# danielmtzbarba/carlabev-env

Measured on NVIDIA B200. Metric: env-steps/sec (obs+reward+done) at N envs, 1/2/4/8 B200; % HBM roofline, higher is better.
Workload: dtype f64

## Files before the change

### carlabev_env_b200/csrc/api.cu

```cuda
#include <cuda.h>
#include <math.h>
#include <stdarg.h>
#include <stdio.h>
#include <stdlib.h>
#include <string.h>

#include <algorithm>
#include <chrono>
#include <cmath>
#include <new>
#include <random>
#include <vector>

#include "engine.h"

static thread_local char g_err[512] = "";

void cbev_set_error(const char* fmt, ...) {
  va_list ap;
  va_start(ap, fmt);
  vsnprintf(g_err, sizeof(g_err), fmt, ap);
  va_end(ap);
}

// ... 344 lines not shown
  else e->frame_bytes = (int64_t)cfg->fov_size * cfg->fov_size * 3;

  const size_t N = (size_t)e->N, A = (size_t)(cfg->max_actors > 0 ? cfg->max_actors : 1);
  int rc = 0;
  rc |= dev_alloc(&e->st.scene, N);
  rc |= dev_alloc(&e->st.episode, N);
  rc |= dev_alloc(&e->st.done, N);
  rc |= dev_alloc(&e->st.ego, N * 24);
  rc |= dev_alloc(&e->st.egoi, N * 8);
  rc |= dev_alloc(&e->st.tgt_vis, N * CBEV_TGT_WORDS);
  rc |= dev_alloc(&e->st.stats, N * 12);
  rc |= dev_alloc(&e->st.ax, N * A);
  rc |= dev_alloc(&e->st.ay, N * A);
  rc |= dev_alloc(&e->st.ayaw, N * A);
  rc |= dev_alloc(&e->st.av, N * A);
  rc |= dev_alloc(&e->st.atarget_mps, N * A);
  rc |= dev_alloc(&e->st.aelapsed, N * A);
  rc |= dev_alloc(&e->st.astate_elapsed, N * A);
  rc |= dev_alloc(&e->st.atidx, N * A);
  rc |= dev_alloc(&e->st.arxlen, N * A);
  rc |= dev_alloc(&e->st.aflags, N * A);
  rc |= dev_alloc(&e->desc, N * CBEV_DESC_WORDS);
  rc |= dev_alloc(&e->order, N);
  rc |= dev_alloc(&e->order_cnt, (size_t)2);
  rc |= dev_alloc(&e->move_order, N);
  rc |= dev_alloc(&e->move_cnt, (size_t)2);
  rc |= dev_alloc(&e->fov, N * (size_t)cfg->fov_size * cfg->fov_size);
  rc |= dev_alloc(&e->gstats, (size_t)CBEV_STATS_FIELDS);
  rc |= build_resize_tables(e);
  rc |= dev_alloc((uint8_t**)&e->h_reward_dev, N * 10);
  e->h_term_dev = (uint8_t*)e->h_reward_dev + N * 8;
  e->h_trunc_dev = e->h_term_dev + N;
  rc |= dev_alloc((uint8_t**)&e->h_actions_dev, N * 16);
  if (rc) { cbev_destroy(e); return rc; }
  cudaMemset(e->st.scene, 0xff, N * sizeof(int32_t));
  {
    uint64_t z = (uint64_t)std::chrono::steady_clock::now().time_since_epoch().count() ^ (uint64_t)(uintptr_t)e;
    try {
      std::random_device rd;
      z ^= ((uint64_t)rd() << 32) | (uint64_t)rd();
    } catch (...) {
    }
    z += 0x9E3779B97F4A7C15ull;
    z = (z ^ (z >> 30)) * 0xBF58476D1CE4E5B9ull;
    z = (z ^ (z >> 27)) * 0x94D049BB133111EBull;
    e->token = z ^ (z >> 31);
  }
  *out = e;
  return CBEV_OK;
}

int cbev_destroy(cbev_handle e) {
  if (!e) return CBEV_OK;
  use_device(e);
  free_pool(e->pool);
  free_state(e->st);
  free_state(e->branch);
  dev_free(e->br_stage_desc); dev_free(e->br_stage_rects); dev_free(e->br_desc); dev_free(e->br_rects);
  dev_free(e->br_window);
  dev_free(e->fov_mask); dev_free(e->rs_tab); dev_free(e->trace);
  dev_free(e->order); dev_free(e->order_cnt); dev_free(e->move_order); dev_free(e->move_cnt);
  dev_free(e->map); dev_free(e->desc); dev_free(e->rects); dev_free(e->fov); dev_free(e->gstats);
  dev_free(e->h_reward_dev);
  { uint8_t* p = (uint8_t*)e->h_actions_dev; dev_free(p); }
  if (e->side_stream) cudaStreamDestroy(e->side_stream);
  if (e->ev_sim) cudaEventDestroy(e->ev_sim);
  if (e->ev_copy) cudaEventDestroy(e->ev_copy);
  if (e->ev_judge) cudaEventDestroy(e->ev_judge);
  if (e->prof_ev) {
    for (int i = 0; i < CBEV_PROF_EVENTS * CBEV_PROF_MAX; ++i) cudaEventDestroy(e->prof_ev[i]);
    delete[] e->prof_ev;
  }
  delete e;
  return CBEV_OK;
}

int cbev_upload_map(cbev_handle e, const uint8_t* cls_host, int32_t w, int32_t h_px) {
  if (!e || !cls_host) { cbev_set_error("null argument"); return CBEV_ERR_ARG; }
  { int rc0 = use_device(e); if (rc0) return rc0; }
  if (w < 16 || h_px < 16 || (w % 16) != 0) { cbev_set_error("map width must be a multiple of 16 (TMA row pitch), got %dx%d", w, h_px); return CBEV_ERR_ARG; }
  for (size_t i = 0; i < (size_t)w * h_px; ++i)
    if (cls_host[i] > 2) { cbev_set_error("map classes must be 0 (non-drivable), 1 (drivable) or 2 (sidewalk)"); return CBEV_ERR_ARG; }
  dev_free(e->map);
  int rc = dev_upload(&e->map, cls_host, (size_t)w * h_px);
// ... 798 lines not shown
    std::vector<int32_t> ti(N * A);
    std::vector<uint8_t> fl(N * A);
    for (size_t i = 0; i < N * A; ++i) {
      const double* o = actors_host + i * 8;
      x[i] = o[0]; y[i] = o[1]; yaw[i] = o[2]; v[i] = o[3];
      ti[i] = (int32_t)o[4];
      tm[i] = o[6];
      fl[i] = (uint8_t)(((int)o[7] & ~15) | ((int)o[5] & 15));
    }
    CU_TRY(cudaMemcpy(e->st.ax, x.data(), N * A * 8, cudaMemcpyHostToDevice));
    CU_TRY(cudaMemcpy(e->st.ay, y.data(), N * A * 8, cudaMemcpyHostToDevice));
    CU_TRY(cudaMemcpy(e->st.ayaw, yaw.data(), N * A * 8, cudaMemcpyHostToDevice));
    CU_TRY(cudaMemcpy(e->st.av, v.data(), N * A * 8, cudaMemcpyHostToDevice));
    CU_TRY(cudaMemcpy(e->st.atarget_mps, tm.data(), N * A * 8, cudaMemcpyHostToDevice));
    CU_TRY(cudaMemcpy(e->st.atidx, ti.data(), N * A * 4, cudaMemcpyHostToDevice));
    CU_TRY(cudaMemcpy(e->st.aflags, fl.data(), N * A, cudaMemcpyHostToDevice));
  }
  return CBEV_OK;
}

int cbev_set_debug_flags(cbev_handle e, int32_t flags) {
  if (!e) { cbev_set_error("null handle"); return CBEV_ERR_ARG; }
  if (flags & ~CBEV_DBG_KNOWN) {
    cbev_set_error("unknown debug flags 0x%x (accepted bits: 1, 2, 4, 32, 128, 256, 512)",
                   (unsigned)(flags & ~CBEV_DBG_KNOWN));
    return CBEV_ERR_ARG;
  }
  e->debug_flags = flags;
  if ((flags & CBEV_DBG_TRACE) && !e->trace) return dev_alloc(&e->trace, (size_t)e->N * 8);
  return CBEV_OK;
}

int cbev_debug_read_trace(cbev_handle e, uint64_t* host_out) {
  if (!e || !host_out) { cbev_set_error("null argument"); return CBEV_ERR_ARG; }
  { int rc0 = use_device(e); if (rc0) return rc0; }
  if (!e->trace) { cbev_set_error("tracing is off (set debug flag 4 first)"); return CBEV_ERR_STATE; }
  CU_TRY(cudaDeviceSynchronize());
  CU_TRY(cudaMemcpy(host_out, e->trace, (size_t)e->N * 8 * sizeof(uint64_t), cudaMemcpyDeviceToHost));
  return CBEV_OK;
}

int cbev_keep_fov(cbev_handle e, int32_t on) {
  if (!e) { cbev_set_error("null handle"); return CBEV_ERR_ARG; }
  e->keep_fov = on != 0;
  return CBEV_OK;
}

int cbev_copy_fov(cbev_handle e, uint8_t* fov_dev, void* stream) {
  if (!e || !fov_dev) { cbev_set_error("null argument"); return CBEV_ERR_ARG; }
  { int rc0 = use_device(e); if (rc0) return rc0; }
  if (!e->keep_fov) { cbev_set_error("palette frames are not kept: call cbev_keep_fov(h, 1) before stepping"); return CBEV_ERR_STATE; }
  size_t bytes = (size_t)e->N * e->cfg.fov_size * e->cfg.fov_size;
  CU_TRY(cudaMemcpyAsync(fov_dev, e->fov, bytes, cudaMemcpyDeviceToDevice, (cudaStream_t)stream));
  return CBEV_OK;
}

int cbev_read_stats(cbev_handle e, double* stats_dev, int32_t reset_after, void* stream) {
  if (!e || !stats_dev) { cbev_set_error("null argument"); return CBEV_ERR_ARG; }
  { int rc0 = use_device(e); if (rc0) return rc0; }
// ... 64 lines not shown
```

### carlabev_env_b200/csrc/engine.h

```cpp
#pragma once
#include <cuda_runtime.h>
#include <stdint.h>

#include "../../include/cbev.h"

#define CBEV_TGT_WORDS 2
#define CBEV_MAX_TARGETS (64 * CBEV_TGT_WORDS)
#define CBEV_RECT_WORDS 2
#define CBEV_DESC_WORDS 20
#define CBEV_TILE_H 184
#define CBEV_TILE_W 208
#define CBEV_WARPS_PER_BLOCK 4
#define CBEV_PROF_MAX 2048
#define CBEV_PROF_EVENTS 5

enum {
  RD_OX = 0,
  RD_OY,
  RD_MODE,
  RD_TURNS,
  RD_NX, RD_NY, RD_ISIN, RD_ICOS, RD_AX, RD_AY, RD_XD, RD_YD, RD_CY,
  RD_NRECTS,
  RD_FLAGS,
  RD_FX, RD_FY,
// ... 70 lines not shown
  float hero_scale;
  int32_t action_mode, n_discrete, reward_mode, autoreset;
  uint64_t seed;
  const uint8_t* map;
  float discrete_table[16 * 3];
  cbev_config cfg;
};

#define CBEV_RS_FAST96 0
#define CBEV_RS_TABLE 1
#define CBEV_RS_HALF 2
#define CBEV_RS_COPY 3
#define CBEV_RS_LINEAR 4
#define CBEV_ANY_BOX_W 128

enum {
  CBEV_DBG_GENERIC_ROTATE = 1,
  CBEV_DBG_JUDGE_SERIAL = 2,
  CBEV_DBG_TRACE = 4,
  CBEV_DBG_IDENTITY_RENDER_ORDER = 32,
  CBEV_DBG_IDENTITY_MOVE_ORDER = 128,
  CBEV_DBG_RENDER_ANY = 256,
  CBEV_DBG_NO_BLOCK83 = 512,
  CBEV_DBG_KNOWN = CBEV_DBG_GENERIC_ROTATE | CBEV_DBG_JUDGE_SERIAL | CBEV_DBG_TRACE | CBEV_DBG_IDENTITY_RENDER_ORDER |
                   CBEV_DBG_IDENTITY_MOVE_ORDER | CBEV_DBG_RENDER_ANY | CBEV_DBG_NO_BLOCK83
};

struct cbev_engine {
  cbev_config cfg;
  int device = 0;
  int32_t N = 0, crop = 0, pad = 0, anchor_x = 0, anchor_y = 0;
  int32_t map_w = 0, map_h = 0;
  uint8_t* map = nullptr;
  alignas(64) unsigned char tmap[128];
  alignas(64) unsigned char tmap_any[128];
  int32_t win_max = 0;
  int32_t any_nbx = 0, any_nby = 0, any_box_h = 0;
  bool has_map = false, has_pool = false, was_reset = false, keep_fov = false;
  PoolDev pool;
  EnvState st;
  int32_t max_rects = 0;
  int32_t debug_flags = 0;
  int32_t* desc = nullptr;
  uint32_t* rects = nullptr;
  int32_t* order = nullptr;
  int32_t* order_cnt = nullptr;
  int32_t* move_order = nullptr;
  int32_t* move_cnt = nullptr;
  uint8_t* fov = nullptr;
  unsigned long long* trace = nullptr;
  int32_t rs_mode = 0, rs_words = 0;
  int32_t* rs_tab = nullptr;
  uint8_t* fov_mask = nullptr;
  void* ring = nullptr;
  int64_t ring_bytes = 0, frame_bytes = 0;
  int32_t channels = 0;
  int32_t head = -1;
  double* gstats = nullptr;
  void* h_actions_dev = nullptr;
  double* h_reward_dev = nullptr;
  uint8_t *h_term_dev = nullptr, *h_trunc_dev = nullptr;
  cudaStream_t side_stream = nullptr;
  cudaEvent_t ev_sim = nullptr, ev_copy = nullptr, ev_judge = nullptr;
  bool host_copy_pending = false;
  int64_t launches = 0;
  int64_t steps = 0;
  bool profiling = false;
  cudaEvent_t* prof_ev = nullptr;
  int32_t prof_n = 0;
// ... 46 lines not shown
```

### carlabev_env_b200/csrc/render.cu

```cuda
#include <cuda.h>
#include <stdlib.h>

#include <type_traits>

#include "engine.h"

namespace {

constexpr int RT = 256;

__constant__ uint32_t c_pal_rg[CBEV_PAL_COUNT];
__constant__ uint32_t c_pal_b[CBEV_PAL_COUNT];
__constant__ uint32_t c_pal_key[CBEV_PAL_COUNT];
__constant__ uint8_t c_chan_mask[6][CBEV_PAL_COUNT + 1];

__device__ __forceinline__ uint32_t smem_u32(const void* p) { return (uint32_t)__cvta_generic_to_shared(p); }

__device__ __forceinline__ void mbar_init(uint64_t* bar, int count) {
  asm volatile("mbarrier.init.shared::cta.b64 [%0], %1;" ::"r"(smem_u32(bar)), "r"(count));
}
__device__ __forceinline__ void mbar_expect_tx(uint64_t* bar, uint32_t bytes) {
  asm volatile("mbarrier.arrive.expect_tx.shared::cta.b64 _, [%0], %1;" ::"r"(smem_u32(bar)), "r"(bytes) : "memory");
}
__device__ __forceinline__ void mbar_wait(uint64_t* bar, uint32_t parity) {
// ... 22 lines not shown
__device__ __forceinline__ uint32_t bit_to_f32(uint32_t m, int pos) {
  int32_t s;
  asm("bfe.s32 %0, %1, %2, 1;" : "=r"(s) : "r"(m), "r"(pos));
  return (uint32_t)s & 0x3f800000u;
}
__device__ __forceinline__ void st_b4(void* p, uint32_t a, uint32_t b, uint32_t c, uint32_t d) {
  asm volatile("st.global.cs.v4.b32 [%0], {%1, %2, %3, %4};" ::"l"(p), "r"(a), "r"(b), "r"(c), "r"(d) : "memory");
}
__device__ __forceinline__ void st_u4(void* p, uint4 v) {
  asm volatile("st.global.cs.v4.u32 [%0], {%1, %2, %3, %4};" ::"l"(p), "r"(v.x), "r"(v.y), "r"(v.z), "r"(v.w)
               : "memory");
}

struct RenderParams {
  int32_t N, fov, crop, anchor_x, anchor_y;
  int32_t frame_stack, ring_slots, head, mirror;
  int64_t frame_bytes;
  int32_t generic_rotate;
  int32_t blk83;
  int32_t list_cap;
  const int32_t* desc;
  const uint32_t* rects;
  const int32_t* order;
  int32_t* order_cnt;
  int32_t max_rects;
  uint8_t* fov_out;
  const uint8_t* fov_mask;
  void* ring;
  int32_t obs_h, obs_w, rs_mode, rs_words;
  const int32_t* rs_tab;
  unsigned long long* trace;
  int32_t hero_w;
  int32_t nbx, nby, box_h, region_bytes;
};

__device__ __forceinline__ void trace_mark(const RenderParams& P, int env, int slot) {
  if (P.trace != nullptr && threadIdx.x == 0) {
    unsigned long long t;
    asm volatile("mov.u64 %0, %%globaltimer;" : "=l"(t));
    P.trace[(size_t)env * 8 + slot] = t;
    if (slot == 0) {
      unsigned sm;
      asm volatile("mov.u32 %0, %%smid;" : "=r"(sm));
      P.trace[(size_t)env * 8 + 6] = sm;
    }
  }
}
// ... 65 lines not shown

template <int OBS_MODE, int CHANNELS, bool U8 = false>
__global__ void __launch_bounds__(RT, 4)
k_render(RenderParams P, const __grid_constant__ CUtensorMap tmap, int mask_mode) {
  extern __shared__ __align__(128) uint8_t smem[];
  constexpr int S = 128;
  constexpr int pitch = CBEV_TILE_W;
  constexpr int tile_bytes = CBEV_TILE_W * CBEV_TILE_H;
  uint8_t* s_tile = smem;
  uint8_t* const s_region = smem;
  uint8_t* s_fov = smem + tile_bytes;
  uint32_t* s_rg = (uint32_t*)(s_fov + S * S);
  uint32_t* s_b = s_rg + 16;
  uint32_t* s_key = s_b + 16;
  int32_t* s_desc = (int32_t*)(s_key + 16);
  uint64_t* s_bar = (uint64_t*)(s_desc + CBEV_DESC_WORDS);
  uint8_t* s_cm = (uint8_t*)(s_bar + 2);
  int* s_count = (int*)(s_cm + 16);
  uint32_t* s_rects = (uint32_t*)(s_count + 4);

  const int env = P.order != nullptr ? P.order[blockIdx.x] : blockIdx.x;
  const int tid = threadIdx.x;
  const int lane = tid & 31, warp = tid >> 5;
  if (blockIdx.x == 0 && tid < 2 && P.order_cnt != nullptr) P.order_cnt[tid] = 0;
  const int32_t* d = P.desc + (size_t)env * CBEV_DESC_WORDS;
  const int flags = d[RD_FLAGS];
  if (flags & 2) return;
  trace_mark(P, env, 0);

  if (tid == 0) {
    mbar_init(s_bar, 1);
    asm volatile("fence.mbarrier_init.release.cluster;" ::: "memory");
    mbar_expect_tx(s_bar, (uint32_t)tile_bytes);
    tma_load_2d(s_tile, &tmap, d[RD_OX] & ~15, d[RD_OY], s_bar);
    *s_count = 0;
  }
  if (tid < CBEV_DESC_WORDS) s_desc[tid] = d[tid];
  if (tid < CBEV_PAL_COUNT) {
    s_rg[tid] = c_pal_rg[tid];
    s_b[tid] = c_pal_b[tid];
    s_key[tid] = c_pal_key[tid];
  }
  if (tid <= CBEV_PAL_COUNT) s_cm[tid] = c_chan_mask[mask_mode][tid];
  const int nrects = d[RD_NRECTS];
  {
    const uint32_t* rl = P.rects + (size_t)env * P.max_rects * CBEV_RECT_WORDS;
    for (int r = tid; r < P.max_rects * CBEV_RECT_WORDS; r += RT) s_rects[r] = rl[r];
// ... 271 lines not shown
  const int S = P.fov, NT = blockDim.x;
  const int FP = S + 16;
  constexpr int BW = CBEV_ANY_BOX_W;
  const int tile_h = P.box_h * P.nby;
  const int tile_bytes = BW * P.nbx * tile_h;
  uint8_t* const s_tile = smem;
  uint8_t* const s_fov = smem + P.region_bytes;
  uint32_t* s_rg = (uint32_t*)(s_fov + S * FP);
  uint32_t* s_b = s_rg + 16;
  uint32_t* s_key = s_b + 16;
  int32_t* s_desc = (int32_t*)(s_key + 16);
  uint64_t* s_bar = (uint64_t*)(s_desc + CBEV_DESC_WORDS);
  uint8_t* s_cm = (uint8_t*)(s_bar + 2);
  uint8_t* s_cmu = s_cm + 16;
  float4* s_palf = (float4*)(s_cmu + 16);
  uint32_t* s_rects = (uint32_t*)(s_palf + 16);
  int32_t* s_tab = (int32_t*)(s_rects + ((P.max_rects * CBEV_RECT_WORDS + 3) & ~3));
  uint8_t* s_bflag = (uint8_t*)(s_tab + P.rs_words);
  uint8_t* s_out_sep = s_bflag + ((((S >> 3) * (S >> 3)) + 15) & ~15);

  const int env = P.order != nullptr ? P.order[blockIdx.x] : blockIdx.x;
  const int tid = threadIdx.x;
  const int lane = tid & 31, warp = tid >> 5, nwarps = NT >> 5;
  if (blockIdx.x == 0 && tid < 2 && P.order_cnt != nullptr) P.order_cnt[tid] = 0;
  const int32_t* d = P.desc + (size_t)env * CBEV_DESC_WORDS;
  const int flags = d[RD_FLAGS];
  if (flags & 2) return;
  trace_mark(P, env, 0);

  if (tid == 0) {
    mbar_init(s_bar, 1);
    asm volatile("fence.mbarrier_init.release.cluster;" ::: "memory");
    mbar_expect_tx(s_bar, (uint32_t)tile_bytes);
    const int x0 = d[RD_OX] & ~15, y0 = d[RD_OY];
    for (int bx = 0; bx < P.nbx; ++bx)
      for (int by = 0; by < P.nby; ++by)
        tma_load_2d(s_tile + (size_t)(bx * tile_h + by * P.box_h) * BW, &tmap, x0 + bx * BW, y0 + by * P.box_h, s_bar);
  }
  if (tid < CBEV_DESC_WORDS) s_desc[tid] = d[tid];
  if (tid < CBEV_PAL_COUNT) {
    s_rg[tid] = c_pal_rg[tid];
    s_b[tid] = c_pal_b[tid];
    s_key[tid] = c_pal_key[tid];
  }
  if (tid <= CBEV_PAL_COUNT) s_cm[tid] = c_chan_mask[mask_mode][tid];
  const int nrects = d[RD_NRECTS];
  {
// ... 641 lines not shown
                   e->max_rects);
    return 1;
  }
  int rc = 1;
  if (e->cfg.obs_mode == CBEV_OBS_RGB) rc = launch<CBEV_OBS_RGB, 1>(e, P, smem, smem_any, any, s);
  else if (e->cfg.obs_mode == CBEV_OBS_GRAY) rc = launch<CBEV_OBS_GRAY, 1>(e, P, smem, smem_any, any, s);
  else if (e->cfg.obs_mode == CBEV_OBS_SEMANTIC_U8) rc = launch_semantic<true>(e, P, smem, smem_any, any, s);
  else rc = launch_semantic<false>(e, P, smem, smem_any, any, s);
  if (rc == 0) e->launches += 1;
  return rc;
}

}

int cbev_launch_render(cbev_engine* e, int32_t head, int32_t mirror, cudaStream_t s) {
  RenderParams P;
  P.N = e->N;
  P.ring_slots = e->cfg.ring_slots;
  P.head = head;
  P.mirror = mirror;
  P.desc = e->desc;
  P.rects = e->rects;
  P.order = (e->debug_flags & CBEV_DBG_IDENTITY_RENDER_ORDER) ? nullptr : e->order;
  P.order_cnt = e->order_cnt;
  P.fov_out = e->keep_fov ? e->fov : nullptr;
  P.ring = e->ring;
  P.trace = (e->debug_flags & CBEV_DBG_TRACE) ? e->trace : nullptr;
  return render_launch(e, P, s);
}

int cbev_launch_render_branches(cbev_engine* e, int32_t n, void* windows, cudaStream_t s) {
  RenderParams P;
  P.N = n;
  P.ring_slots = 1;
  P.head = 0;
  P.mirror = 0;
  P.desc = e->br_desc;
  P.rects = e->br_rects;
  P.order = nullptr;
  P.order_cnt = nullptr;
  P.fov_out = nullptr;
  P.ring = windows;
  P.trace = nullptr;
  return render_launch(e, P, s);
}

int cbev_launch_fuse(cbev_engine* e, int32_t mode, const void* ring, int32_t n, int32_t L, int32_t head, void* out,
                     cudaStream_t s) {
  static const int veh_of[6] = {-1, -1, 1, 2, 3, 3};
  const int veh = veh_of[e->cfg.mask_mode];
  if (veh < 0) return 1;
  const int C = e->channels;
  const int Cout = mode == CBEV_FUSE_VEHICLE_TEMPORAL ? C - 1 + 3 : C;
  const bool u8 = e->cfg.obs_mode == CBEV_OBS_SEMANTIC_U8;
  const int HWV = e->cfg.obs_h * e->cfg.obs_w / (u8 ? 16 : 4);
  long long total = (long long)n * Cout * HWV;
  int blocks = (int)((total + 255) / 256);
  if (blocks > 148 * 32) blocks = 148 * 32;
  if (!u8)
    k_fuse<<<blocks, 256, 0, s>>>((const float4*)ring, (float*)out, n, L, C, head, veh, mode, HWV);
  else if (mode == CBEV_FUSE_VEHICLE_TEMPORAL)
    k_fuse<<<blocks, 256, 0, s>>>((const uint4*)ring, (uint8_t*)out, n, L, C, head, veh, mode, HWV);
  else
// ... 5 lines not shown
```

### carlabev_env_b200/csrc/sim.cu

```cuda
#include <limits.h>
#include <math.h>

#include "engine.h"

#ifndef CBEV_SIM_BLOCKS_PER_SM
#define CBEV_SIM_BLOCKS_PER_SM 7
#endif

namespace {

constexpr double DT = 0.1;
constexpr double WB = 2.9;
constexpr double KST = 2.0;
constexpr double KPS = 1.0;
constexpr double MPP = 0.3125;
constexpr double MAX_STEER = 0x1.0c152382d7365p-1;
constexpr double PI = 0x1.921fb54442d18p+1;
constexpr double TWO_PI = 0x1.921fb54442d18p+2;
constexpr double HALF_PI = 0x1.921fb54442d18p+0;
constexpr double DEG2RAD = 0x1.1df46a2529d39p-6;
constexpr double RAD2DEG = 0x1.ca5dc1a63c1f8p+5;
constexpr unsigned FULL = 0xffffffffu;

enum { E_X = 0, E_Y, E_YAW, E_V, E_X1, E_Y1, E_YAW1, E_V1, E_ACC, E_T, E_D2G, E_D2G1, E_SPREV, E_LAST_DYAW,
// ... 495 lines not shown
__device__ __forceinline__ void live_actor_chunk(const SimParams& P, const PoolDev& pool, const EnvState& S, size_t row, int ga,
                                              size_t o, bool has, double t_sim, int lane, int gb, unsigned GM, Body& b,
                                              int& kind) {
  actor_chunk_step<G>(P, pool, S, row, ga, o, has, t_sim, lane, gb, GM, b, kind);
}

template <int G>
__device__ __forceinline__ void hand_over_to_live(const SimParams& P, const PoolDev& pool, const EnvState& st, int env, int scene,
                                               int A, int lane, unsigned GM) {
  for (int a = lane; a < A; a += G) {
    const size_t o = (size_t)env * P.max_actors + a, r = (size_t)scene * P.max_actors + a;
    st.ax[o] = pool.roll.ax[r]; st.ay[o] = pool.roll.ay[r]; st.ayaw[o] = pool.roll.ayaw[r]; st.av[o] = pool.roll.av[r];
    st.atarget_mps[o] = pool.roll.atarget_mps[r]; st.aelapsed[o] = pool.roll.aelapsed[r];
    st.astate_elapsed[o] = pool.roll.astate_elapsed[r]; st.atidx[o] = pool.roll.atidx[r];
    st.arxlen[o] = pool.roll.arxlen[r]; st.aflags[o] = pool.roll.aflags[r];
  }
  for (int k = lane; k < P.max_retreat * 3 * CBEV_SG_MAX; k += G)
    st.retreat[(size_t)env * P.max_retreat * 3 * CBEV_SG_MAX + k] = pool.roll.retreat[(size_t)scene * P.max_retreat * 3 * CBEV_SG_MAX + k];
  for (int k = lane; k < P.max_retreat; k += G)
    st.retreat_n[(size_t)env * P.max_retreat + k] = pool.roll.retreat_n[(size_t)scene * P.max_retreat + k];
  __syncwarp(GM);
}

template <int G>
__device__ __forceinline__ void auto_reset_env(const SimParams& P, const PoolDev& pool, const EnvState& st, const cbev_step_out& out,
                                            int32_t* d, int32_t* order, int32_t* order_cnt, int env, int lane, unsigned GM) {
  int ep = st.episode[env];
  uint64_t h = splitmix64(P.seed + (uint64_t)env * 0x9E3779B97F4A7C15ull + (uint64_t)ep * 0xD1B54A32D192ED03ull);
  int scene = (int)(h % (uint64_t)pool.n_scenes);
  __syncwarp(GM);
  reset_env(P, pool, st, env, scene, lane, G);
  if (lane == 0) {
    order[atomicAdd(order_cnt, 1)] = env;
    const double* s0 = pool.ego_state0 + (size_t)scene * 4;
    View v;
    compute_view(P, s0[0], s0[1], 0.0, v);
    write_desc_header(P, d, v, 0, 1, crop_corner_class(P, v));
    out.reward[env] = 0.0;
    out.terminated[env] = 0;
    out.truncated[env] = 0;
    if (out.cause) out.cause[env] = CBEV_CAUSE_NONE;
    if (out.hero) {
      double* hb = out.hero + (size_t)env * CBEV_HERO_FIELDS;
      for (int k = 0; k < CBEV_HERO_FIELDS; ++k) hb[k] = 0.0;
      hb[CBEV_H_X] = s0[0]; hb[CBEV_H_Y] = s0[1]; hb[CBEV_H_YAW] = s0[2]; hb[CBEV_H_V] = s0[3];
      hb[CBEV_H_SCENE] = (double)scene;
    }
  }
}

template <int G>
struct Group {
  int warp, lane, gb, grp;
  unsigned GM;
  int env;
  __device__ __forceinline__ Group(const SimParams& P, const int32_t* __restrict__ perm = nullptr) {
    constexpr int EPW = 32 / G;
    warp = threadIdx.x >> 5;
    const int wl = threadIdx.x & 31;
    lane = wl & (G - 1);
    gb = wl & ~(G - 1);
    grp = wl / G;
    GM = G == 32 ? 0xffffffffu : (((1u << G) - 1u) << gb);
    env = (blockIdx.x * CBEV_WARPS_PER_BLOCK + warp) * EPW + grp;
    if (perm != nullptr && env < P.N) env = perm[env];
  }
};

enum { MV_LIVE = 0, MV_BRANCH = 1, MV_BRANCH_DRAW = 2 };
template <int G, int MODE>
__device__ __forceinline__ void move_body(const SimParams& P, const PoolDev& pool, const EnvState& st,
                                          const void* __restrict__ actions, const cbev_step_out& out,
                                          int32_t* __restrict__ desc, uint32_t* __restrict__ rects,
                                          int32_t* __restrict__ order, int32_t* __restrict__ order_cnt, int env,
                                          int lane, int gb, unsigned GM) {
  constexpr bool BRANCH = MODE != MV_LIVE, DRAW = MODE != MV_BRANCH;
  int32_t* d = desc + (size_t)env * CBEV_DESC_WORDS;
  uint32_t* rl = rects + (size_t)env * P.max_rects * CBEV_RECT_WORDS;

  const uint8_t was_done = BRANCH ? 0 : st.done[env];
  const int scene = st.scene[env];
  double* eg = st.ego + (size_t)env * E_SLOTS;
  const int32_t* ei = st.egoi + (size_t)env * I_SLOTS;
  Body e;
  e.x = eg[E_X]; e.y = eg[E_Y]; e.yaw = eg[E_YAW]; e.v = eg[E_V];
  double acc = eg[E_ACC];
  const double etarget = eg[E_TARGET];
  const double t_sim = eg[E_T] + DT;
  const int step_idx = ei[I_STEP];
  const unsigned long long tv0 = st.tgt_vis[(size_t)env * CBEV_TGT_WORDS], tv1 = st.tgt_vis[(size_t)env * CBEV_TGT_WORDS + 1];
  float gas, steer, brake;
  if (P.action_mode == CBEV_ACTION_DISCRETE) {
    long long id = ((const long long*)actions)[env];
    const int nd = P.n_discrete;
    id = id < 0 ? 0 : (id >= nd ? nd - 1 : id);
    gas = P.discrete_table[id * 3 + 0];
    steer = P.discrete_table[id * 3 + 1];
    brake = P.discrete_table[id * 3 + 2];
  } else {
    const float* a = (const float*)actions + (size_t)env * 3;
    gas = fminf(fmaxf(a[0], 0.0f), 1.0f);
    steer = fminf(fmaxf(a[1], -1.0f), 1.0f);
    brake = fminf(fmaxf(a[2], 0.0f), 1.0f);
  }

  if constexpr (!BRANCH) {
    if (P.autoreset == CBEV_AUTORESET_NEXT_STEP && was_done) {
      auto_reset_env<G>(P, pool, st, out, d, order, order_cnt, env, lane, GM);
      return;
    }
  }

  const int r0 = pool.ego_off[scene], nt = pool.ego_off[scene + 1] - r0;
  const int A0 = pool.actor_off[scene], A = pool.actor_off[scene + 1] - A0;
  const int tl0 = pool.tl_off[scene], ntl = pool.tl_off[scene + 1] - tl0;
  const bool use_table = step_idx < pool.traj_steps;
  const long long toff = pool.traj_steps > 0 ? pool.traj_off[scene] : 0;
  const double* __restrict__ ecx = pool.ego_cx + r0;
  const double* __restrict__ ecy = pool.ego_cy + r0;

  double acc_val = gas > 0.0f ? (double)__fmul_rn(gas, P.hero_scale) : 0.0;
  double delta;
  if (fabs(e.v) < 0.1) {
    delta = 0.0;
  } else {
    double steer_deg = clipd(18.0 / (1.0 + 0.35 * fabs(e.v)), 8.0, 18.0);
    delta = ((double)steer * steer_deg) * DEG2RAD;
  }
  double speed_factor = clipd(fabs(e.v) / 5.0, 0.3, 1.0);
  double brake_val = (brake > 0.0f ? (double)__fmul_rn(__fmul_rn(brake, 0.6f), P.hero_scale) : 0.0) * speed_factor;
  double target_acc = acc_val - brake_val - 0.05 * e.v;
  acc = (1.0 - 0.2) * acc + 0.2 * target_acc;
  const double applied_delta = delta;
  body_update(e, acc, delta, etarget);
  e.v *= 0.9999;
  if (fabs(e.v) < 0.05) e.v = 0.0;
  e.v *= 0.985;
  if (lane == 0) {
    eg[E_X] = e.x; eg[E_Y] = e.y; eg[E_YAW] = e.yaw; eg[E_V] = e.v;
    eg[E_X1] = e.x1; eg[E_Y1] = e.y1; eg[E_YAW1] = e.yaw1; eg[E_V1] = e.v1;
    eg[E_ACC] = acc;
    eg[E_GAS] = (double)gas; eg[E_STEER] = (double)steer; eg[E_BRAKE] = (double)brake; eg[E_DELTA] = applied_delta;
  }

  const int pad = P.pad;
  View view;
  int bg = 0;
  if constexpr (DRAW) {
    compute_view(P, e.x, e.y, e.yaw, view);
    bg = crop_corner_class(P, view);
  }

  int nrects = 0;
  if (!use_table && pool.traj_steps > 0 && step_idx == pool.traj_steps) hand_over_to_live<G>(P, pool, st, env, scene, A, lane, GM);
  double4 qn = make_double4(0.0, 0.0, 0.0, 0.0);
  int kn = 0;
  if (use_table && lane < A) {
    qn = pool.traj[toff + (size_t)step_idx * A + lane];
    kn = pool.act_kind[A0 + lane];
  }
  for (int base = 0; base < A; base += G) {
    const int a = base + lane;
    const bool has = a < A;
    const int ga = A0 + (has ? a : 0);
    const size_t o = (size_t)env * P.max_actors + (has ? a : 0);
    Body b;
    int kind = 0;
    if (use_table) {
      const double4 q = qn;
      kind = kn;
      if (a + G < A) {
        qn = pool.traj[toff + (size_t)step_idx * A + a + G];
        kn = pool.act_kind[ga + G];
      }
      if (has) {
        b.x = q.x; b.y = q.y; b.yaw = q.z; b.v = q.w;
        st.ax[o] = b.x; st.ay[o] = b.y; st.ayaw[o] = b.yaw; st.av[o] = b.v;
      }
    } else {
      live_actor_chunk<G>(P, pool, st, (size_t)env, ga, o, has, t_sim, lane, gb, GM, b, kind);
    }
    if constexpr (!DRAW) continue;
    const int size = kind == 0 ? 4 : 2;
    uint32_t pk0 = 0, pk1 = 0;
    bool vis = false, c00 = false;
    const int pal = kind == 0 ? CBEV_PAL_VEHICLE : CBEV_PAL_PEDESTRIAN;
    if (has) {
      const int rx = rect_left(b.x, pad, size), ry = rect_left(b.y, pad, size);
      vis = pack_rect(rx, ry, size, size, pal, view, pk0, pk1, c00);
    }
    {
      unsigned bm = __ballot_sync(GM, c00) >> gb;
      if (bm) bg = __shfl_sync(GM, pal, gb + 31 - __clz(bm));
    }
    unsigned vm = __ballot_sync(GM, vis) >> gb;
    if (vis) {
      uint32_t* w = rl + (size_t)(nrects + __popc(vm & ((1u << lane) - 1u))) * CBEV_RECT_WORDS;
      w[0] = pk0; w[1] = pk1;
    }
    nrects += __popc(vm);
  }
  if constexpr (DRAW) {
    for (int base = 0; base < nt; base += G) {
      int i = base + lane;
      bool has = i < nt && ((((i >> 6) ? tv1 : tv0) >> (i & 63)) & 1ull);
      int size = (i == nt - 1) ? 4 : 2;
      uint32_t pk0 = 0, pk1 = 0;
      bool vis = false, c00 = false;
      if (has) {
        const int tx = rect_left(ecx[i], pad, size), ty = rect_left(ecy[i], pad, size);
        vis = pack_rect(tx, ty, size, size, CBEV_PAL_ROUTE, view, pk0, pk1, c00);
      }
      if (__ballot_sync(GM, c00)) bg = CBEV_PAL_ROUTE;
      unsigned vm = __ballot_sync(GM, vis) >> gb;
      if (vis) {
        uint32_t* w = rl + (size_t)(nrects + __popc(vm & ((1u << lane) - 1u))) * CBEV_RECT_WORDS;
        w[0] = pk0; w[1] = pk1;
      }
      nrects += __popc(vm);
    }
    {
      const int t0 = tl0;
      for (int base = 0; base < ntl; base += G) {
        int i = base + lane;
        uint32_t pk0 = 0, pk1 = 0;
        bool vis = false, c00 = false;
        int pal = 0;
        if (i < ntl) {
          const int32_t* r = pool.tl_rect + (size_t)(t0 + i) * 4;
          pal = pool.tl_color[t0 + i];
          vis = pack_rect(r[0], r[1], r[2], r[3], pal, view, pk0, pk1, c00);
        }
        {
          unsigned bm = __ballot_sync(GM, c00) >> gb;
          if (bm) bg = __shfl_sync(GM, pal, gb + 31 - __clz(bm));
        }
        unsigned vm = __ballot_sync(GM, vis) >> gb;
        if (vis) {
          uint32_t* w = rl + (size_t)(nrects + __popc(vm & ((1u << lane) - 1u))) * CBEV_RECT_WORDS;
          w[0] = pk0; w[1] = pk1;
        }
        nrects += __popc(vm);
      }
    }
    if (lane == 0) {
      write_desc_header(P, d, view, nrects, 0, bg);
      if constexpr (!BRANCH) order[P.N - 1 - atomicAdd(order_cnt + 1, 1)] = env;
    }
  }
}

template <int G>
__global__ void __launch_bounds__(32 * CBEV_WARPS_PER_BLOCK, G == 32 ? CBEV_SIM_BLOCKS_PER_SM : 4)
k_move(SimParams P, PoolDev pool, EnvState st, const void* __restrict__ actions, cbev_step_out out,
       int32_t* __restrict__ desc, uint32_t* __restrict__ rects, int32_t* __restrict__ order,
       int32_t* __restrict__ order_cnt, const int32_t* __restrict__ move_order, int32_t* __restrict__ move_cnt) {
  const Group<G> g(P, move_order);
  if (blockIdx.x == 0 && threadIdx.x < 2 && move_cnt != nullptr) move_cnt[threadIdx.x] = 0;
  if (g.env >= P.N) return;
  move_body<G, MV_LIVE>(P, pool, st, actions, out, desc, rects, order, order_cnt, g.env, g.lane, g.gb, g.GM);
}

enum { JG_LIVE = 0, JG_BRANCH = 1, JG_BRANCH_ROW = 2 };
template <int G, int MODE>
__device__ __forceinline__ void judge_body(const SimParams& P, const PoolDev& pool, const EnvState& st,
                                           const cbev_step_out& out, double* __restrict__ gstats,
                                           int32_t* __restrict__ move_order, int32_t* __restrict__ move_cnt,
                                           double* __restrict__ hb_s, int env, int lane, int gb, unsigned GM, bool last,
                                           double& reward_out, bool& terminated_out, bool& truncated_out,
                                           int& cause_out) {
  constexpr bool BRANCH = MODE != JG_LIVE;
  const int scene = st.scene[env];
  const int r0 = pool.ego_off[scene], nt = pool.ego_off[scene + 1] - r0;
  const double* __restrict__ ecx = pool.ego_cx + r0;
  const double* __restrict__ ecy = pool.ego_cy + r0;
  const double* __restrict__ ecyaw = pool.ego_cyaw + r0;
  double* eg = st.ego + (size_t)env * E_SLOTS;
  int32_t* ei = st.egoi + (size_t)env * I_SLOTS;

  Body e;
  e.x = eg[E_X]; e.y = eg[E_Y]; e.yaw = eg[E_YAW]; e.v = eg[E_V];
  e.x1 = eg[E_X1]; e.y1 = eg[E_Y1]; e.yaw1 = eg[E_YAW1]; e.v1 = eg[E_V1];
  const double acc = eg[E_ACC];
// ... 327 lines not shown
      hb[CBEV_H_DIST2GOAL] = d2g; hb[CBEV_H_T] = t_sim; hb[CBEV_H_SCENE] = (double)scene;
    }
  }
  __syncwarp(GM);
  if (hero_now) {
    for (int f = lane; f < CBEV_HERO_FIELDS; f += G) out.hero[(size_t)env * CBEV_HERO_FIELDS + f] = hb_s[f];
  }
  reward_out = reward;
  terminated_out = terminated;
  truncated_out = truncated;
  cause_out = cause;
}

template <int G>
__global__ void __launch_bounds__(32 * CBEV_WARPS_PER_BLOCK, 4)
k_judge(SimParams P, PoolDev pool, EnvState st, cbev_step_out out, const int32_t* __restrict__ desc,
        double* __restrict__ gstats, int32_t* __restrict__ move_order, int32_t* __restrict__ move_cnt) {
  constexpr int EPW = 32 / G;
  __shared__ double s_hero[CBEV_WARPS_PER_BLOCK][EPW][CBEV_HERO_FIELDS];
  const Group<G> g(P);
  const int lane = g.lane, env = g.env;
  if (env >= P.N) return;
  if (desc[(size_t)env * CBEV_DESC_WORDS + RD_FLAGS] & 1) {
    if (lane == 0) move_order[P.N - 1 - atomicAdd(move_cnt + 1, 1)] = env;
    return;
  }
  double reward;
  bool terminated, truncated;
  int cause;
  judge_body<G, JG_LIVE>(P, pool, st, out, gstats, move_order, move_cnt, s_hero[g.warp][g.grp], env, lane, g.gb, g.GM,
                       false, reward, terminated, truncated, cause);
}

__global__ void __launch_bounds__(32 * CBEV_WARPS_PER_BLOCK)
k_rollout(SimParams P, PoolDev pool) {
  const int scene = blockIdx.x * CBEV_WARPS_PER_BLOCK + (threadIdx.x >> 5);
  const int lane = threadIdx.x & 31;
  if (scene >= pool.n_scenes) return;
  const int A0 = pool.actor_off[scene], A = pool.actor_off[scene + 1] - A0;
  init_actors(P, pool, pool.roll, (size_t)scene, scene, lane, 32);
  __syncwarp();
  double t_sim = 0.0;
  for (int step = 0; step < pool.traj_steps; ++step) {
    t_sim += DT;
    for (int base = 0; base < A; base += 32) {
      const int a = base + lane;
// ... 92 lines not shown
        const uint8_t* sp = a.src[s] + (size_t)root * n * es;
        for (int i = lane; i < n; i += G) cbev_copy_elem(dp + (size_t)i * es, sp + (size_t)i * es, es);
      }
    }
  }
  if constexpr (LEAF) {
    if (!valid && lane == 0) br.scene[b] = -1;
  }
  __syncwarp(GM);
  const cbev_lookahead_out& o = a.out;
  cbev_step_out so = {};
  so.hero = o.hero;
  double ret = 0.0, w = 1.0;
  int steps = 0, cause = CBEV_CAUSE_NONE;
  bool terminated = false, truncated = false;
  if (live) {
    int slot = 0;
    for (int t = 0; t < H; ++t) {
      const void* act = P.action_mode == CBEV_ACTION_DISCRETE
                            ? (const void*)((const long long*)a.actions + (size_t)t * B)
                            : (const void*)((const float*)a.actions + (size_t)t * B * 3);
      if constexpr (OBS) {
        move_body<G, MV_BRANCH_DRAW>(P, pool, br, act, so, rd.stage_desc + (size_t)slot * B * CBEV_DESC_WORDS,
                                     rd.stage_rects + (size_t)slot * B * P.max_rects * CBEV_RECT_WORDS, nullptr,
                                     nullptr, b, lane, g.gb, GM);
        slot = slot + 1 == rd.F ? 0 : slot + 1;
      } else {
        move_body<G, MV_BRANCH>(P, pool, br, act, so, nullptr, nullptr, nullptr, nullptr, b, lane, g.gb, GM);
      }
      __syncwarp(GM);
      double r;
      judge_body<G, LEAF ? JG_BRANCH_ROW : JG_BRANCH>(P, pool, br, so, nullptr, nullptr, nullptr,
                                                      s_hero[g.warp][g.grp], b, lane, g.gb, GM, t == H - 1, r,
                                                      terminated, truncated, cause);
      if (lane == 0 && o.reward) o.reward[(size_t)t * B + b] = r;
      ret = __dadd_rn(ret, __dmul_rn(w, r));
      w = __dmul_rn(w, a.gamma);
      steps = t + 1;
      if (terminated || truncated) break;
    }
  }
  if (o.reward)
    for (int t = steps + lane; t < H; t += G) o.reward[(size_t)t * B + b] = 0.0;
  if (steps == 0 && o.hero)
    for (int f = lane; f < CBEV_HERO_FIELDS; f += G) o.hero[(size_t)b * CBEV_HERO_FIELDS + f] = 0.0;
  if (lane == 0) {
    o.ret[b] = ret;
    if (o.steps) o.steps[b] = steps;
    if (o.terminated) o.terminated[b] = terminated;
    if (o.truncated) o.truncated[b] = truncated;
    if (o.cause) o.cause[b] = (uint8_t)cause;
// ... 60 lines not shown
  P.reward_mode = e->cfg.reward_mode;
  P.autoreset = e->cfg.autoreset;
  P.seed = e->cfg.seed;
  P.map = e->map;
  for (int i = 0; i < 48; ++i) P.discrete_table[i] = e->cfg.discrete_table[i];
  P.cfg = e->cfg;
  return P;
}

void cbev_launch_reset(cbev_engine* e, const uint8_t* mask, const int32_t* scene_ids, cudaStream_t s) {
  SimParams P = make_params(e);
  int blocks = (e->N + CBEV_WARPS_PER_BLOCK - 1) / CBEV_WARPS_PER_BLOCK;
  k_reset<<<blocks, 32 * CBEV_WARPS_PER_BLOCK, 0, s>>>(P, e->pool, e->st, mask, scene_ids, e->desc, e->order, e->move_order);
  e->launches += 1;
}

static bool narrow_groups(const cbev_engine* e) {
  return e->pool.max_actors <= 8 || e->pool.traj_steps > 0;
}

void cbev_launch_move(cbev_engine* e, const void* actions, const cbev_step_out* out, cudaStream_t s) {
  SimParams P = make_params(e);
  const int32_t* mo = (e->debug_flags & CBEV_DBG_IDENTITY_MOVE_ORDER) ? nullptr : e->move_order;
  if (narrow_groups(e)) {
    constexpr int G = 8;
    int per_block = CBEV_WARPS_PER_BLOCK * (32 / G);
    int blocks = (e->N + per_block - 1) / per_block;
    k_move<G><<<blocks, 32 * CBEV_WARPS_PER_BLOCK, 0, s>>>(P, e->pool, e->st, actions, *out, e->desc, e->rects, e->order,
                                                           e->order_cnt, mo, e->move_cnt);
  } else {
    int blocks = (e->N + CBEV_WARPS_PER_BLOCK - 1) / CBEV_WARPS_PER_BLOCK;
    k_move<32><<<blocks, 32 * CBEV_WARPS_PER_BLOCK, 0, s>>>(P, e->pool, e->st, actions, *out, e->desc, e->rects, e->order,
                                                            e->order_cnt, mo, e->move_cnt);
  }
  e->launches += 1;
}

void cbev_launch_judge(cbev_engine* e, const cbev_step_out* out, cudaStream_t s) {
  SimParams P = make_params(e);
  constexpr int G = 8;
  int per_block = CBEV_WARPS_PER_BLOCK * (32 / G);
  int blocks = (e->N + per_block - 1) / per_block;
  k_judge<G><<<blocks, 32 * CBEV_WARPS_PER_BLOCK, 0, s>>>(P, e->pool, e->st, *out, e->desc, e->gstats, e->move_order,
                                                          e->move_cnt);
  e->launches += 1;
}

template <int G>
static void launch_lookahead(int blocks, cudaStream_t s, bool record, bool rows, bool leaf, const SimParams& P,
                             cbev_engine* e, const LookaheadArgs& a, const LookaheadRender& rd,
                             const LookaheadRoots& rr) {
  constexpr int T = 32 * CBEV_WARPS_PER_BLOCK;
  if (!rows && !leaf) {
    if (record) k_lookahead_obs<G><<<blocks, T, 0, s>>>(P, e->pool, e->branch, a, rd);
    else k_lookahead<G><<<blocks, T, 0, s>>>(P, e->pool, e->branch, a);
  } else if (leaf) {
// ... 61 lines not shown
```

Baseline: 21.79 million.

## Move autoreset into judge kernel and drop atomic render-order counters

```diff
diff --git a/carlabev_env_b200/csrc/api.cu b/carlabev_env_b200/csrc/api.cu
--- a/carlabev_env_b200/csrc/api.cu
+++ b/carlabev_env_b200/csrc/api.cu
@@ -390,7 +390,6 @@
   rc |= dev_alloc(&e->st.aflags, N * A);
   rc |= dev_alloc(&e->desc, N * CBEV_DESC_WORDS);
   rc |= dev_alloc(&e->order, N);
-  rc |= dev_alloc(&e->order_cnt, (size_t)2);
   rc |= dev_alloc(&e->move_order, N);
   rc |= dev_alloc(&e->move_cnt, (size_t)2);
   rc |= dev_alloc(&e->fov, N * (size_t)cfg->fov_size * cfg->fov_size);
@@ -427,7 +426,7 @@
   dev_free(e->br_stage_desc); dev_free(e->br_stage_rects); dev_free(e->br_desc); dev_free(e->br_rects);
   dev_free(e->br_window);
   dev_free(e->fov_mask); dev_free(e->rs_tab); dev_free(e->trace);
-  dev_free(e->order); dev_free(e->order_cnt); dev_free(e->move_order); dev_free(e->move_cnt);
+  dev_free(e->order); dev_free(e->move_order); dev_free(e->move_cnt);
   dev_free(e->map); dev_free(e->desc); dev_free(e->rects); dev_free(e->fov); dev_free(e->gstats);
   dev_free(e->h_reward_dev);
   { uint8_t* p = (uint8_t*)e->h_actions_dev; dev_free(p); }
@@ -1272,19 +1271,19 @@
 int cbev_set_debug_flags(cbev_handle e, int32_t flags) {
   if (!e) { cbev_set_error("null handle"); return CBEV_ERR_ARG; }
   if (flags & ~CBEV_DBG_KNOWN) {
-    cbev_set_error("unknown debug flags 0x%x (accepted bits: 1, 2, 4, 32, 128, 256, 512)",
+    cbev_set_error("unknown debug flags 0x%x (accepted bits: 1, 2, 4, 32, 128, 256, 512, 2048)",
                    (unsigned)(flags & ~CBEV_DBG_KNOWN));
     return CBEV_ERR_ARG;
   }
   e->debug_flags = flags;
-  if ((flags & CBEV_DBG_TRACE) && !e->trace) return dev_alloc(&e->trace, (size_t)e->N * 8);
+  if ((flags & (CBEV_DBG_TRACE | CBEV_DBG_MOVE_TRACE)) && !e->trace) return dev_alloc(&e->trace, (size_t)e->N * 8);
   return CBEV_OK;
 }
 
 int cbev_debug_read_trace(cbev_handle e, uint64_t* host_out) {
   if (!e || !host_out) { cbev_set_error("null argument"); return CBEV_ERR_ARG; }
   { int rc0 = use_device(e); if (rc0) return rc0; }
-  if (!e->trace) { cbev_set_error("tracing is off (set debug flag 4 first)"); return CBEV_ERR_STATE; }
+  if (!e->trace) { cbev_set_error("tracing is off (set debug flag 4 or 2048 first)"); return CBEV_ERR_STATE; }
   CU_TRY(cudaDeviceSynchronize());
   CU_TRY(cudaMemcpy(host_out, e->trace, (size_t)e->N * 8 * sizeof(uint64_t), cudaMemcpyDeviceToHost));
   return CBEV_OK;
diff --git a/carlabev_env_b200/csrc/engine.h b/carlabev_env_b200/csrc/engine.h
--- a/carlabev_env_b200/csrc/engine.h
+++ b/carlabev_env_b200/csrc/engine.h
@@ -116,8 +116,9 @@
   CBEV_DBG_IDENTITY_MOVE_ORDER = 128,
   CBEV_DBG_RENDER_ANY = 256,
   CBEV_DBG_NO_BLOCK83 = 512,
+  CBEV_DBG_MOVE_TRACE = 2048,
   CBEV_DBG_KNOWN = CBEV_DBG_GENERIC_ROTATE | CBEV_DBG_JUDGE_SERIAL | CBEV_DBG_TRACE | CBEV_DBG_IDENTITY_RENDER_ORDER |
-                   CBEV_DBG_IDENTITY_MOVE_ORDER | CBEV_DBG_RENDER_ANY | CBEV_DBG_NO_BLOCK83
+                   CBEV_DBG_IDENTITY_MOVE_ORDER | CBEV_DBG_RENDER_ANY | CBEV_DBG_NO_BLOCK83 | CBEV_DBG_MOVE_TRACE
 };
 
 struct cbev_engine {
@@ -138,7 +139,6 @@
   int32_t* desc = nullptr;
   uint32_t* rects = nullptr;
   int32_t* order = nullptr;
-  int32_t* order_cnt = nullptr;
   int32_t* move_order = nullptr;
   int32_t* move_cnt = nullptr;
   uint8_t* fov = nullptr;
diff --git a/carlabev_env_b200/csrc/render.cu b/carlabev_env_b200/csrc/render.cu
--- a/carlabev_env_b200/csrc/render.cu
+++ b/carlabev_env_b200/csrc/render.cu
@@ -68,7 +68,6 @@
   const int32_t* desc;
   const uint32_t* rects;
   const int32_t* order;
-  int32_t* order_cnt;
   int32_t max_rects;
   uint8_t* fov_out;
   const uint8_t* fov_mask;
@@ -180,7 +179,6 @@
   const int env = P.order != nullptr ? P.order[blockIdx.x] : blockIdx.x;
   const int tid = threadIdx.x;
   const int lane = tid & 31, warp = tid >> 5;
-  if (blockIdx.x == 0 && tid < 2 && P.order_cnt != nullptr) P.order_cnt[tid] = 0;
   const int32_t* d = P.desc + (size_t)env * CBEV_DESC_WORDS;
   const int flags = d[RD_FLAGS];
   if (flags & 2) return;
@@ -498,7 +496,6 @@
   const int env = P.order != nullptr ? P.order[blockIdx.x] : blockIdx.x;
   const int tid = threadIdx.x;
   const int lane = tid & 31, warp = tid >> 5, nwarps = NT >> 5;
-  if (blockIdx.x == 0 && tid < 2 && P.order_cnt != nullptr) P.order_cnt[tid] = 0;
   const int32_t* d = P.desc + (size_t)env * CBEV_DESC_WORDS;
   const int flags = d[RD_FLAGS];
   if (flags & 2) return;
@@ -1186,10 +1183,9 @@
   P.desc = e->desc;
   P.rects = e->rects;
   P.order = (e->debug_flags & CBEV_DBG_IDENTITY_RENDER_ORDER) ? nullptr : e->order;
-  P.order_cnt = e->order_cnt;
   P.fov_out = e->keep_fov ? e->fov : nullptr;
   P.ring = e->ring;
-  P.trace = (e->debug_flags & CBEV_DBG_TRACE) ? e->trace : nullptr;
+  P.trace = (e->debug_flags & CBEV_DBG_TRACE) && !(e->debug_flags & CBEV_DBG_MOVE_TRACE) ? e->trace : nullptr;
   return render_launch(e, P, s);
 }
 
@@ -1202,7 +1198,6 @@
   P.desc = e->br_desc;
   P.rects = e->br_rects;
   P.order = nullptr;
-  P.order_cnt = nullptr;
   P.fov_out = nullptr;
   P.ring = windows;
   P.trace = nullptr;
diff --git a/carlabev_env_b200/csrc/sim.cu b/carlabev_env_b200/csrc/sim.cu
--- a/carlabev_env_b200/csrc/sim.cu
+++ b/carlabev_env_b200/csrc/sim.cu
@@ -541,20 +541,28 @@
   __syncwarp(GM);
 }
 
+__device__ __forceinline__ int auto_reset_scene(const SimParams& P, const PoolDev& pool, const EnvState& st, int env) {
+  const int ep = st.episode[env];
+  const uint64_t h = splitmix64(P.seed + (uint64_t)env * 0x9E3779B97F4A7C15ull + (uint64_t)ep * 0xD1B54A32D192ED03ull);
+  return (int)(h % (uint64_t)pool.n_scenes);
+}
+
+__device__ __forceinline__ void auto_reset_desc(const SimParams& P, const PoolDev& pool, const EnvState& st, int32_t* d,
+                                                int env) {
+  const double* s0 = pool.ego_state0 + (size_t)auto_reset_scene(P, pool, st, env) * 4;
+  View v;
+  compute_view(P, s0[0], s0[1], 0.0, v);
+  write_desc_header(P, d, v, 0, 1, crop_corner_class(P, v));
+}
+
 template <int G>
-__device__ __forceinline__ void auto_reset_env(const SimParams& P, const PoolDev& pool, const EnvState& st, const cbev_step_out& out,
-                                            int32_t* d, int32_t* order, int32_t* order_cnt, int env, int lane, unsigned GM) {
-  int ep = st.episode[env];
-  uint64_t h = splitmix64(P.seed + (uint64_t)env * 0x9E3779B97F4A7C15ull + (uint64_t)ep * 0xD1B54A32D192ED03ull);
-  int scene = (int)(h % (uint64_t)pool.n_scenes);
+__device__ __forceinline__ void auto_reset_env(const SimParams& P, const PoolDev& pool, const EnvState& st,
+                                               const cbev_step_out& out, int env, int lane, unsigned GM) {
+  const int scene = auto_reset_scene(P, pool, st, env);
   __syncwarp(GM);
   reset_env(P, pool, st, env, scene, lane, G);
   if (lane == 0) {
-    order[atomicAdd(order_cnt, 1)] = env;
     const double* s0 = pool.ego_state0 + (size_t)scene * 4;
-    View v;
-    compute_view(P, s0[0], s0[1], 0.0, v);
-    write_desc_header(P, d, v, 0, 1, crop_corner_class(P, v));
     out.reward[env] = 0.0;
     out.terminated[env] = 0;
     out.truncated[env] = 0;
@@ -587,13 +595,51 @@
 };
 
 enum { MV_LIVE = 0, MV_BRANCH = 1, MV_BRANCH_DRAW = 2 };
-template <int G, int MODE>
+
+struct MoveTrace {
+  unsigned long long* row;
+  long long c0;
+  __device__ __forceinline__ static unsigned long long gtime() {
+    unsigned long long t;
+    asm volatile("mov.u64 %0, %%globaltimer;" : "=l"(t)::"memory");
+    return t;
+  }
+  __device__ __forceinline__ static long long clk() {
+    long long c;
+    asm volatile("mov.u64 %0, %%clock64;" : "=l"(c)::"memory");
+    return c;
+  }
+  __device__ __forceinline__ void start(unsigned long long* tr, int env, int lane) {
+    row = tr + (size_t)env * 8;
+    c0 = clk();
+    if (lane == 0) row[0] = gtime();
+  }
+  __device__ __forceinline__ void mark(int slot, int lane) {
+    const long long c = clk();
+    if (lane == 0) row[slot] = (unsigned long long)(c - c0);
+  }
+  __device__ __forceinline__ void finish(int lane, unsigned bits, int nrects) {
+    const long long c = clk();
+    const unsigned long long t = gtime();
+    unsigned sm;
+    asm volatile("mov.u32 %0, %%smid;" : "=r"(sm));
+    if (lane == 0) {
+      row[6] = (unsigned long long)(c - c0);
+      row[1] = t;
+      row[7] = bits | (sm << 8) | ((unsigned long long)nrects << 16);
+    }
+  }
+};
+
+template <int G, int MODE, bool TRACE = false>
 __device__ __forceinline__ void move_body(const SimParams& P, const PoolDev& pool, const EnvState& st,
                                           const void* __restrict__ actions, const cbev_step_out& out,
                                           int32_t* __restrict__ desc, uint32_t* __restrict__ rects,
-                                          int32_t* __restrict__ order, int32_t* __restrict__ order_cnt, int env,
-                                          int lane, int gb, unsigned GM) {
+                                          int32_t* __restrict__ order_slot, int env, int lane, int gb, unsigned GM,
+                                          unsigned long long* __restrict__ tr = nullptr) {
   constexpr bool BRANCH = MODE != MV_LIVE, DRAW = MODE != MV_BRANCH;
+  MoveTrace mt;
+  if constexpr (TRACE) mt.start(tr, env, lane);
   int32_t* d = desc + (size_t)env * CBEV_DESC_WORDS;
   uint32_t* rl = rects + (size_t)env * P.max_rects * CBEV_RECT_WORDS;
 
@@ -625,7 +671,14 @@
 
   if constexpr (!BRANCH) {
     if (P.autoreset == CBEV_AUTORESET_NEXT_STEP && was_done) {
-      auto_reset_env<G>(P, pool, st, out, d, order, order_cnt, env, lane, GM);
+      if (lane == 0) {
+        *order_slot = env;
+        auto_reset_desc(P, pool, st, d, env);
+      }
+      if constexpr (TRACE) {
+        mt.mark(2, lane); mt.mark(3, lane); mt.mark(4, lane); mt.mark(5, lane);
+        mt.finish(lane, 1u, 0);
+      }
       return;
     }
   }
@@ -661,6 +714,7 @@
     eg[E_ACC] = acc;
     eg[E_GAS] = (double)gas; eg[E_STEER] = (double)steer; eg[E_BRAKE] = (double)brake; eg[E_DELTA] = applied_delta;
   }
+  if constexpr (TRACE) mt.mark(2, lane);
 
   const int pad = P.pad;
   View view;
@@ -669,6 +723,7 @@
     compute_view(P, e.x, e.y, e.yaw, view);
     bg = crop_corner_class(P, view);
   }
+  if constexpr (TRACE) mt.mark(3, lane);
 
   int nrects = 0;
   if (!use_table && pool.traj_steps > 0 && step_idx == pool.traj_steps) hand_over_to_live<G>(P, pool, st, env, scene, A, lane, GM);
@@ -678,6 +733,8 @@
     qn = pool.traj[toff + (size_t)step_idx * A + lane];
     kn = pool.act_kind[A0 + lane];
   }
+  double tcx = 0.0, tcy = 0.0;
+  if (!BRANCH && lane < nt) { tcx = ecx[lane]; tcy = ecy[lane]; }
   for (int base = 0; base < A; base += G) {
     const int a = base + lane;
     const bool has = a < A;
@@ -719,6 +776,7 @@
     }
     nrects += __popc(vm);
   }
+  if constexpr (TRACE) mt.mark(4, lane);
   if constexpr (DRAW) {
     for (int base = 0; base < nt; base += G) {
       int i = base + lane;
@@ -727,7 +785,8 @@
       uint32_t pk0 = 0, pk1 = 0;
       bool vis = false, c00 = false;
       if (has) {
-        const int tx = rect_left(ecx[i], pad, size), ty = rect_left(ecy[i], pad, size);
+        const bool pre = !BRANCH && base == 0;
+        const int tx = rect_left(pre ? tcx : ecx[i], pad, size), ty = rect_left(pre ? tcy : ecy[i], pad, size);
         vis = pack_rect(tx, ty, size, size, CBEV_PAL_ROUTE, view, pk0, pk1, c00);
       }
       if (__ballot_sync(GM, c00)) bg = CBEV_PAL_ROUTE;
@@ -738,6 +797,7 @@
       }
       nrects += __popc(vm);
     }
+    if constexpr (TRACE) mt.mark(5, lane);
     {
       const int t0 = tl0;
       for (int base = 0; base < ntl; base += G) {
@@ -764,20 +824,22 @@
     }
     if (lane == 0) {
       write_desc_header(P, d, view, nrects, 0, bg);
-      if constexpr (!BRANCH) order[P.N - 1 - atomicAdd(order_cnt + 1, 1)] = env;
-    }
-  }
-}
-
-template <int G>
+      if constexpr (!BRANCH) *order_slot = env;
+    }
+    if constexpr (TRACE) mt.finish(lane, use_table ? 2u : 4u, nrects);
+  }
+}
+
+template <int G, bool TRACE>
 __global__ void __launch_bounds__(32 * CBEV_WARPS_PER_BLOCK, G == 32 ? CBEV_SIM_BLOCKS_PER_SM : 4)
 k_move(SimParams P, PoolDev pool, EnvState st, const void* __restrict__ actions, cbev_step_out out,
        int32_t* __restrict__ desc, uint32_t* __restrict__ rects, int32_t* __restrict__ order,
-       int32_t* __restrict__ order_cnt, const int32_t* __restrict__ move_order, int32_t* __restrict__ move_cnt) {
+       const int32_t* __restrict__ move_order, int32_t* __restrict__ move_cnt, unsigned long long* __restrict__ trace) {
   const Group<G> g(P, move_order);
   if (blockIdx.x == 0 && threadIdx.x < 2 && move_cnt != nullptr) move_cnt[threadIdx.x] = 0;
   if (g.env >= P.N) return;
-  move_body<G, MV_LIVE>(P, pool, st, actions, out, desc, rects, order, order_cnt, g.env, g.lane, g.gb, g.GM);
+  const int gi = (blockIdx.x * CBEV_WARPS_PER_BLOCK + g.warp) * (32 / G) + g.grp;
+  move_body<G, MV_LIVE, TRACE>(P, pool, st, actions, out, desc, rects, order + gi, g.env, g.lane, g.gb, g.GM, trace);
 }
 
 enum { JG_LIVE = 0, JG_BRANCH = 1, JG_BRANCH_ROW = 2 };
@@ -1151,6 +1213,7 @@
   const int lane = g.lane, env = g.env;
   if (env >= P.N) return;
   if (desc[(size_t)env * CBEV_DESC_WORDS + RD_FLAGS] & 1) {
+    auto_reset_env<G>(P, pool, st, out, env, lane, g.GM);
     if (lane == 0) move_order[P.N - 1 - atomicAdd(move_cnt + 1, 1)] = env;
     return;
   }
@@ -1289,11 +1352,11 @@
                             : (const void*)((const float*)a.actions + (size_t)t * B * 3);
       if constexpr (OBS) {
         move_body<G, MV_BRANCH_DRAW>(P, pool, br, act, so, rd.stage_desc + (size_t)slot * B * CBEV_DESC_WORDS,
-                                     rd.stage_rects + (size_t)slot * B * P.max_rects * CBEV_RECT_WORDS, nullptr,
-                                     nullptr, b, lane, g.gb, GM);
+                                     rd.stage_rects + (size_t)slot * B * P.max_rects * CBEV_RECT_WORDS, nullptr, b,
+                                     lane, g.gb, GM);
         slot = slot + 1 == rd.F ? 0 : slot + 1;
       } else {
-        move_body<G, MV_BRANCH>(P, pool, br, act, so, nullptr, nullptr, nullptr, nullptr, b, lane, g.gb, GM);
+        move_body<G, MV_BRANCH>(P, pool, br, act, so, nullptr, nullptr, nullptr, b, lane, g.gb, GM);
       }
       __syncwarp(GM);
       double r;
@@ -1400,16 +1463,18 @@
 void cbev_launch_move(cbev_engine* e, const void* actions, const cbev_step_out* out, cudaStream_t s) {
   SimParams P = make_params(e);
   const int32_t* mo = (e->debug_flags & CBEV_DBG_IDENTITY_MOVE_ORDER) ? nullptr : e->move_order;
+  unsigned long long* tr = (e->debug_flags & CBEV_DBG_MOVE_TRACE) ? e->trace : nullptr;
+  constexpr int T = 32 * CBEV_WARPS_PER_BLOCK;
   if (narrow_groups(e)) {
     constexpr int G = 8;
     int per_block = CBEV_WARPS_PER_BLOCK * (32 / G);
     int blocks = (e->N + per_block - 1) / per_block;
-    k_move<G><<<blocks, 32 * CBEV_WARPS_PER_BLOCK, 0, s>>>(P, e->pool, e->st, actions, *out, e->desc, e->rects, e->order,
-                                                           e->order_cnt, mo, e->move_cnt);
+    if (tr) k_move<G, true><<<blocks, T, 0, s>>>(P, e->pool, e->st, actions, *out, e->desc, e->rects, e->order, mo, e->move_cnt, tr);
+    else k_move<G, false><<<blocks, T, 0, s>>>(P, e->pool, e->st, actions, *out, e->desc, e->rects, e->order, mo, e->move_cnt, tr);
   } else {
     int blocks = (e->N + CBEV_WARPS_PER_BLOCK - 1) / CBEV_WARPS_PER_BLOCK;
-    k_move<32><<<blocks, 32 * CBEV_WARPS_PER_BLOCK, 0, s>>>(P, e->pool, e->st, actions, *out, e->desc, e->rects, e->order,
-                                                            e->order_cnt, mo, e->move_cnt);
+    if (tr) k_move<32, true><<<blocks, T, 0, s>>>(P, e->pool, e->st, actions, *out, e->desc, e->rects, e->order, mo, e->move_cnt, tr);
+    else k_move<32, false><<<blocks, T, 0, s>>>(P, e->pool, e->st, actions, *out, e->desc, e->rects, e->order, mo, e->move_cnt, tr);
   }
   e->launches += 1;
 }
```

Result: faster. 22.03 million, median of 6 (+1.1%).
